# wkentaro/morefusion

Measured on AMD Instinct MI355X. Metric: objects/sec (32^3 voxelize+3D-CNN+ICC refine), higher is better.
Workload: dtype f32; 1 GPU; 1 scene(s) x 8 objects per GPU: singleview_3d Model.predict (ResNet18+PSPNet, 32^3 voxelize, occupancy 3D-CNN, heads; B=8) -> ICC joint refine 100 iters (BASELINE configs[1]+configs[2]); random weights, ICC starts from synthetic perturbed-GT poses; ICC(k) on a second HIP stream, event-ordered after network(k), beside network(k+1); objects_per_gpu=8, icc_iters=100, parallelism=scene-sharded x1, pose all_gather, stream_priority=none, backbone_memory_format=contiguous

## Files before the change

### include/mfhip.h

```cpp
#ifndef MFHIP_H_
#define MFHIP_H_

#include <stdint.h>

#ifdef __cplusplus
extern "C" {
#endif

typedef void *mfStream_t;

int mf_version(void);
const char *mf_last_error_string(void);

int mf_average_voxelization_3d_fwd(const float *values, const float *points,
                                   const int32_t *batch_indices, int64_t n, int C,
                                   int B, int X, int Y, int Z, float ox, float oy,
                                   float oz, float pitch, float *matrix,
                                   int32_t *counts, int32_t *head, int32_t *link,
                                   int32_t *nan_flag, mfStream_t stream);
int mf_average_voxelization_3d_bwd(const float *gmatrix, const float *points,
                                   const int32_t *batch_indices,
                                   const int32_t *counts, int64_t n, int C, int B,
                                   int X, int Y, int Z, float ox, float oy, float oz,
                                   float pitch, float *gvalues, mfStream_t stream);
// ... 217 lines not shown
int64_t mf_sparse_conv3_bf16_workspace_bytes(int64_t n_points, int32_t B, int32_t D);
int mf_sparse_conv3_bf16_tables(void *ws, int64_t n_points, int32_t B, int32_t D, int64_t *out7);
int mf_sparse_conv3_bf16_index(const float *points, const int32_t *batch_indices, int64_t n, int32_t B, int32_t D,
                               void *ws, mfStream_t stream);
int mf_sparse_conv3_bf16_pack(const float *W, int32_t Cout, int32_t Cs, int32_t w_cin, int32_t c_off, void *Wp, void *Wq,
                              mfStream_t stream);
int mf_sparse_conv3_bf16_unpack_dw(const float *dWp, int32_t Cout, int32_t Cs, int32_t w_cin, int32_t c_off, float *dW,
                                   mfStream_t stream);
int mf_sparse_conv3_bf16_reduce(const void *C, const float *dense, const float *bias, void *ws, int64_t n_points,
                                int32_t B, int32_t D, int32_t Cout, int32_t relu, void *out, mfStream_t stream);
int mf_sparse_conv3_bf16_gather_dy(const void *dz, void *ws, int64_t n_points, int32_t B, int32_t D, int32_t Cout,
                                   void *dYg, mfStream_t stream);
int mf_linear_bf16_tiles(const void *A, int32_t lda, const void *W, int64_t w_group_stride, int32_t ldw,
                         const int32_t *tile_group, void *out, int32_t ldo, int32_t M, int32_t N, int32_t K,
                         int32_t out_f32, mfStream_t stream);
int mf_linear_wgrad_bf16_ranges(const void *dY, int32_t ldy, const void *A, int32_t lda, float *dW,
                                int64_t w_group_stride, int32_t ldc, const int32_t *m_range, int32_t groups, int32_t N,
                                int32_t K, mfStream_t stream);
int mf_conv3d_k4s2_bf16_pack_cols(const float *W, int32_t Cout, int32_t Cin, int32_t w_cin, int32_t c_off, void *W2,
                                  mfStream_t stream);
int mf_conv3d_k4s2_bf16_col2im(const void *T, int32_t B, int32_t D, int32_t Cin, void *dx, mfStream_t stream);
int mf_average_voxelization_rows_bf16_fwd(const void *values, int64_t ldv, const float *points,
                                          const int32_t *batch_indices, int64_t n, int32_t C, int32_t B, int32_t D,
                                          const int32_t *counts, const int32_t *head, const int32_t *link,
                                          const int32_t *rowmap, void *A, int64_t lda, mfStream_t stream);
int mf_average_voxelization_rows_bf16_bwd(const void *dA, int64_t lda, const float *points,
                                          const int32_t *batch_indices, const int32_t *counts, const int32_t *rowmap,
                                          int64_t n, int32_t C, int32_t B, int32_t D, void *gvalues, int64_t ldg,
                                          mfStream_t stream);

int mf_average_voxelization_cl_bf16_fwd(const void *values, int64_t ldv, const float *points,
                                        const int32_t *batch_indices, int64_t n, int32_t C, int32_t B, int32_t D,
                                        void *x, int64_t ldx, int32_t *counts, int32_t *head, int32_t *link,
                                        mfStream_t stream);
int mf_average_voxelization_cl_bf16_bwd(const void *gx, int64_t ldx, const float *points, const int32_t *batch_indices,
                                        const int32_t *counts, int64_t n, int32_t C, int32_t B, int32_t D,
                                        void *gvalues, int64_t ldg, mfStream_t stream);
int mf_interpolate_voxel_grid_cl_bf16_fwd(const void *vox, const float *points, const int32_t *batch_indices,
                                          int64_t n, int B, int C, int X, int Y, int Z, void *out, int64_t ldo,
                                          mfStream_t stream);
int mf_interpolate_voxel_grid_cl_bf16_bwd(const void *gout, int64_t ldg, const float *points,
                                          const int32_t *batch_indices, const int32_t *batch_start, int64_t n, int B,
                                          int C, int X, int Y, int Z, void *gvox, int32_t out_bf16, mfStream_t stream);

int mf_upsample_bilinear_cl_fwd(const void *x, void *y, int32_t B, int32_t H, int32_t W, int32_t Ho, int32_t Wo,
                                int32_t C, int32_t bf16, mfStream_t stream);
int mf_upsample_bilinear_cl_split_fwd(const float *x, void *y, int32_t B, int32_t H, int32_t W, int32_t Ho, int32_t Wo,
                                      int32_t C, int32_t ldy, int32_t los, mfStream_t stream);
int mf_split_bf16(const float *x, int64_t sb, int64_t sc, int64_t sh, int64_t sw, int32_t B, int32_t C, int32_t H,
                  int32_t W, void *y, int32_t ldy, int32_t los, mfStream_t stream);
int mf_upsample2x_tapsum_fwd(const float *z, const float *bias, const float *slope, int32_t act, float *y32,
                             int32_t ld32, void *ys, int32_t lds, int32_t los, int32_t B, int32_t H, int32_t W, int32_t C,
                             mfStream_t stream);
int mf_upsample_bilinear_cl_bwd(const void *gy, void *gx, int32_t B, int32_t H, int32_t W, int32_t Ho, int32_t Wo,
                                int32_t C, int32_t bf16, mfStream_t stream);
int mf_upsample_bilinear_cf_fwd(const void *x, void *y, int64_t BC, int32_t H, int32_t W, int32_t Ho, int32_t Wo,
                                int32_t bf16, mfStream_t stream);
int mf_upsample_bilinear_cf_bwd(const void *gy, void *gx, int64_t BC, int32_t H, int32_t W, int32_t Ho, int32_t Wo,
                                int32_t bf16, mfStream_t stream);
int mf_prelu_fwd(const void *x, const float *slope, void *y, int64_t n, int32_t bf16, mfStream_t stream);
int mf_rgb_normalize(const void *rgb, int32_t u8, const float *mean3, const float *std3, float *out, int64_t npix,
                     mfStream_t stream);
int mf_bn_act_fwd(const void *x, const void *identity, const float *mean, const float *var, const float *weight,
                  const float *bias, float eps, void *y, int64_t n, int32_t C, int64_t HW, int32_t channels_last,
                  int32_t relu, int32_t bf16, mfStream_t stream);
int mf_backbone2d_last_path(void);
int64_t mf_prelu_bwd_workspace_floats(int64_t n);
int mf_prelu_bwd(const void *x, const void *dy, const float *slope, void *dx, float *dslope, float *ws, int64_t n,
                 int32_t bf16, mfStream_t stream);

int mf_gemm_bf16_last_tile(void);

int mf_gemm_bf16_nt_plan(int32_t mode, int64_t M, int32_t N, int32_t K, int32_t groups, int32_t table,
                         int64_t dgrad_rows, int32_t may_split, int32_t have_ws, int32_t *tile, int32_t *S);
int mf_gemm_bf16_tn_plan(int32_t Ni, int32_t Nj, int32_t ldc, int64_t rows, int32_t groups, int32_t ranges,
                         int32_t conv, int32_t split, int32_t *form, int32_t *default_split, int32_t *finish);

int mf_psp_tail_rows_bf16_fwd(const void *u2, const int64_t *pix, int32_t B, int32_t P, int32_t H, int32_t W, void *rows,
                              mfStream_t stream);
int mf_psp_tail_rows_bf16_bwd(const void *grows, const int64_t *pix, int32_t B, int32_t P, int32_t H, int32_t W,
                              float *acc, void *gu2, mfStream_t stream);

int mf_confidence_loss_fwd(const float *add, const float *conf, int32_t B, int32_t P, float lambda, float *loss,
                           int32_t *cnt, mfStream_t stream);
int mf_confidence_loss_bwd(const float *add, const float *conf, const int32_t *cnt, const float *gloss, int32_t B,
                           int32_t P, float lambda, float *dadd, float *dconf, mfStream_t stream);

int mf_pose_epilogue_train_fwd(const float *orot, const float *otrn, const float *ocnf, const int64_t *class_id,
                               const float *pts, const float *origin, const float *pitch, int32_t B, int32_t P,
                               int32_t n_fg, float *rot, float *trans, float *conf, mfStream_t stream);
int mf_pose_epilogue_train_bwd(const float *orot, const float *ocnf, const int64_t *class_id, const float *pitch,
                               const float *grot, const float *gtrans, const float *gconf, int32_t B, int32_t P,
                               int32_t n_fg, float *drot, float *dtrn, float *dcnf, mfStream_t stream);
int mf_transformation_matrix_fwd(const float *q, const float *t, int64_t n, float *T, mfStream_t stream);
int mf_transformation_matrix_bwd(const float *q, const float *gT, int64_t n, float *gq, float *gt, mfStream_t stream);
int mf_point_prep(const float *points_cam, const float *values, const float *origin, const float *pitch,
                  int32_t B, int32_t P, int32_t Cv, float center, float *pts, float *tc4, float *x_rows,
                  int32_t *batch_indices, mfStream_t stream);
int mf_pose_epilogue(const float *heads_out, int64_t ldo, int32_t np4, const int64_t *class_id,
                     const float *pts, const float *origin, const float *pitch, int32_t B, int32_t P, int32_t n_fg,
                     float *rot, float *trans, float *conf, mfStream_t stream);

#define MF_PCDNET_WS_BUFFERS 12
#define MF_PCDNET_MAX_FG 256
int32_t mf_pcdnet_workspace_offsets(int32_t B, int32_t P, int32_t n_fg, int64_t *offsets);
int64_t mf_pcdnet_workspace_bytes(int32_t B, int32_t P, int32_t n_fg);
// ... 214 lines not shown
```

### morefusion_amd/_lib.py

```python
import ctypes
import os

import torch

_HERE = os.path.dirname(os.path.abspath(__file__))
SO_PATH = os.path.join(_HERE, os.path.basename(os.environ.get("MF_LIBMFHIP", "libmfhip.so")))
_lib = None

_p = ctypes.c_void_p
_i = ctypes.c_int32
_i64 = ctypes.c_int64
_f = ctypes.c_float
_d = ctypes.c_double


class IccBatch(ctypes.Structure):

    _fields_ = [
        ("pts4", _p), ("obj_off", _p), ("scene_off", _p), ("obj_scene", _p),
        ("pitch", _p), ("origin", _p), ("grid_target", _p), ("grid_ne", _p),
        ("n_objects", _i), ("n_scenes", _i), ("n_points", _i), ("dim", _i), ("max_scene_objects", _i),
        ("voxel_threshold", _f), ("sdf_offset", _f), ("grid_ne_binary", _i), ("flags", _i),
    ]

# ... 78 lines not shown
    "mf_linear_bf16": ([_p, _i64, _i, _p, _i64, _i, _p, _i64, _p, _i64] + [_i] * 8 + [_p], _i),
    "mf_linear_wgrad_bf16": ([_p, _i64, _i, _p, _i64, _i, _p, _i64, _i, _p] + [_i] * 5 + [_p], _i),
    "mf_conv3d_k4s2_pack_bf16": ([_p] + [_i] * 4 + [_p, _p, _p], _i),
    "mf_conv3d_k4s2_bf16_fwd": ([_p, _p, _p, _p] + [_i] * 6 + [_p], _i),
    "mf_conv3d_k4s2_bf16_dgrad": ([_p, _p, _p] + [_i] * 6 + [_p], _i),
    "mf_conv3d_k4s2_bf16_wgrad_workspace_bytes": ([_i] * 3, _i64),
    "mf_conv3d_k4s2_bf16_wgrad_default_split": ([_i] * 4, _i),
    "mf_conv3d_k4s2_bf16_wgrad": ([_p, _p, _p, _p] + [_i] * 7 + [_p], _i),
    "mf_conv3d_bf16_pack": ([_p] + [_i] * 5 + [_p, _p, _p, _p], _i),
    "mf_conv3d_bf16_fwd": ([_p, _p, _p, _p] + [_i] * 11 + [_p], _i),
    "mf_conv3d_bf16_fwd_workspace_bytes": ([_i] * 8, _i64),
    "mf_conv3d_bf16_fwd_ws": ([_p, _p, _p, _p, _p, _i64] + [_i] * 11 + [_p], _i),
    "mf_conv2d_split_pack": ([_p] + [_i] * 3 + [_p, _p], _i),
    "mf_conv2d_split_workspace_bytes": ([_i] * 8, _i64),
    "mf_conv2d_split_fwd": ([_p, _p, _p, _p, _i, _p, _i, _p, _i, _p, _i, _i, _p, _i64] + [_i] * 8 + [_p], _i),
    "mf_conv3d_k4s2_split_pack": ([_p] + [_i] * 4 + [_p, _p], _i),
    "mf_conv3d_k4s2_split_workspace_bytes": ([_i] * 4, _i64),
    "mf_conv3d_k4s2_split_fwd": ([_p, _p, _p, _i, _p, _i, _p, _i, _i, _p, _i64] + [_i] * 4 + [_p], _i),
    "mf_linear_split_pack": ([_p, _i64] + [_i] * 6 + [_p, _p], _i),
    "mf_linear_split_workspace_bytes": ([_i64, _i, _i], _i64),
    "mf_linear_split_fwd": ([_p, _i, _p, _p, _i, _p, _i, _p, _i, _i, _p, _i64] + [_i] * 3 + [_p], _i),
    "mf_sparse_conv3d_k4s2_points_cl_split_fwd": ([_p, _i64, _p, _p, _i64, _f, _f, _f, _f, _p, _p, _p, _p, _p, _p] + [_i] * 6 + [_p], _i),
    "mf_interpolate_voxel_grid_cl_split_fwd": ([_p, _p, _p, _i64, _i, _i, _i, _i, _i, _p, _i64, _i64, _p], _i),
    "mf_conv3d_k3_narrow_bf16_pack_elems": ([_i], _i64),
    "mf_conv3d_k3_narrow_bf16_pack": ([_p] + [_i] * 5 + [_p, _p], _i),
    "mf_conv3d_k3_narrow_bf16": ([_p, _p, _p, _p] + [_i] * 6 + [_p], _i),
    "mf_conv3d_bf16_wgrad_workspace_bytes": ([_i] * 4, _i64),
    "mf_wgrad_split": ([_i64, _i64, _i64], _i),
    "mf_linear_wgrad_bf16_default_split": ([_i64, _i, _i, _i], _i),
    "mf_conv3d_bf16_wgrad_default_split": ([_i] * 5, _i),
    "mf_conv3d_bf16_wgrad": ([_p, _p, _p, _p] + [_i] * 11 + [_p], _i),
    "mf_sparse_conv3_bf16_max_rows": ([_i64], _i64),
    "mf_sparse_conv3_bf16_workspace_bytes": ([_i64, _i, _i], _i64),
    "mf_sparse_conv3_bf16_tables": ([_p, _i64, _i, _i, _p], _i),
    "mf_sparse_conv3_bf16_index": ([_p, _p, _i64, _i, _i, _p, _p], _i),
    "mf_sparse_conv3_bf16_pack": ([_p, _i, _i, _i, _i, _p, _p, _p], _i),
    "mf_sparse_conv3_bf16_unpack_dw": ([_p, _i, _i, _i, _i, _p, _p], _i),
    "mf_sparse_conv3_bf16_reduce": ([_p, _p, _p, _p, _i64, _i, _i, _i, _i, _p, _p], _i),
    "mf_sparse_conv3_bf16_gather_dy": ([_p, _p, _i64, _i, _i, _i, _p, _p], _i),
    "mf_linear_bf16_tiles": ([_p, _i, _p, _i64, _i, _p, _p, _i, _i, _i, _i, _i, _p], _i),
    "mf_linear_wgrad_bf16_ranges": ([_p, _i, _p, _i, _p, _i64, _i, _p, _i, _i, _i, _p], _i),
    "mf_conv3d_k4s2_bf16_pack_cols": ([_p, _i, _i, _i, _i, _p, _p], _i),
    "mf_conv3d_k4s2_bf16_col2im": ([_p, _i, _i, _i, _p, _p], _i),
    "mf_average_voxelization_rows_bf16_fwd": ([_p, _i64, _p, _p, _i64, _i, _i, _i, _p, _p, _p, _p, _p, _i64, _p], _i),
    "mf_average_voxelization_rows_bf16_bwd": ([_p, _i64, _p, _p, _p, _p, _i64, _i, _i, _i, _p, _i64, _p], _i),
    "mf_average_voxelization_cl_bf16_fwd": ([_p, _i64, _p, _p, _i64, _i, _i, _i, _p, _i64, _p, _p, _p, _p], _i),
    "mf_average_voxelization_cl_bf16_bwd": ([_p, _i64, _p, _p, _p, _i64, _i, _i, _i, _p, _i64, _p], _i),
    "mf_interpolate_voxel_grid_cl_bf16_fwd": ([_p, _p, _p, _i64, _i, _i, _i, _i, _i, _p, _i64, _p], _i),
    "mf_interpolate_voxel_grid_cl_bf16_bwd": ([_p, _i64, _p, _p, _p, _i64, _i, _i, _i, _i, _i, _p, _i, _p], _i),
    "mf_upsample_bilinear_cl_fwd": ([_p, _p] + [_i] * 7 + [_p], _i),
    "mf_upsample_bilinear_cl_split_fwd": ([_p, _p] + [_i] * 8 + [_p], _i),
    "mf_upsample2x_tapsum_fwd": ([_p, _p, _p, _i, _p, _i, _p] + [_i] * 6 + [_p], _i),
    "mf_split_bf16": ([_p, _i64, _i64, _i64, _i64] + [_i] * 4 + [_p, _i, _i, _p], _i),
    "mf_upsample_bilinear_cl_bwd": ([_p, _p] + [_i] * 7 + [_p], _i),
    "mf_upsample_bilinear_cf_fwd": ([_p, _p, _i64] + [_i] * 5 + [_p], _i),
    "mf_upsample_bilinear_cf_bwd": ([_p, _p, _i64] + [_i] * 5 + [_p], _i),
    "mf_prelu_fwd": ([_p, _p, _p, _i64, _i, _p], _i),
    "mf_rgb_normalize": ([_p, _i, _p, _p, _p, _i64, _p], _i),
    "mf_bn_act_fwd": ([_p, _p, _p, _p, _p, _p, _f, _p, _i64, _i, _i64, _i, _i, _i, _p], _i),
    "mf_backbone2d_last_path": ([], _i),
    "mf_prelu_bwd_workspace_floats": ([_i64], _i64),
    "mf_prelu_bwd": ([_p, _p, _p, _p, _p, _p, _i64, _i, _p], _i),
    "mf_gemm_bf16_last_tile": ([], _i),
    "mf_gemm_bf16_nt_plan": ([_i, _i64, _i, _i, _i, _i, _i64, _i, _i, _p, _p], _i),
    "mf_gemm_bf16_tn_plan": ([_i, _i, _i, _i64, _i, _i, _i, _i, _p, _p, _p], _i),
    "mf_psp_tail_rows_bf16_fwd": ([_p, _p, _i, _i, _i, _i, _p, _p], _i),
    "mf_psp_tail_rows_bf16_bwd": ([_p, _p, _i, _i, _i, _i, _p, _p, _p], _i),
    "mf_confidence_loss_fwd": ([_p, _p, _i, _i, _f, _p, _p, _p], _i),
    "mf_confidence_loss_bwd": ([_p, _p, _p, _p, _i, _i, _f, _p, _p, _p], _i),
    "mf_pose_epilogue_train_fwd": ([_p, _p, _p, _p, _p, _p, _p, _i, _i, _i, _p, _p, _p, _p], _i),
    "mf_pose_epilogue_train_bwd": ([_p, _p, _p, _p, _p, _p, _p, _i, _i, _i, _p, _p, _p, _p], _i),
    "mf_transformation_matrix_fwd": ([_p, _p, _i64, _p, _p], _i),
    "mf_transformation_matrix_bwd": ([_p, _p, _i64, _p, _p, _p], _i),
    "mf_point_prep": ([_p, _p, _p, _p, _i, _i, _i, _f, _p, _p, _p, _p, _p], _i),
    "mf_pose_epilogue": ([_p, _i64, _i, _p, _p, _p, _p, _i, _i, _i, _p, _p, _p, _p], _i),
    "mf_psp_tail_fwd": ([_p, _i64, _i64, _i64, _i64, _p, _p, _p, _p, _p, _p] + [_i] * 4 + [_p, _p], _i),
    "mf_valid_pixel_order": ([_p, _i, _i, _p, _p, _p], _i),
    "mf_instance_stats": ([_p, _p, _i, _i, _p, _i, _p, _p], _i),
    "mf_instance_crops": ([_p, _p, _p, _i, _i, _d, _d, _d, _d, _p, _p, _i, _i, _i, _p, _p, _p, _p], _i),
    "mf_occmap_regrid": ([ctypes.POINTER(OccTree), ctypes.POINTER(OccTree), _p], _i),
    "mf_occmap_bounds": ([_p, _p, _i64, _p, _i, _p, _i, _p, _p], _i),
    "mf_occmap_raycast": ([_p, _p, _i64, _p, _i, _p, _f, _f, _f, _p, _p], _i),
    "mf_occmap_count_hits": ([_p, _i64, _p, _i, _p, _p], _i),
    "mf_occmap_apply": ([_p, _i, _i64, _i, _p], _i),
    "mf_occmap_extract": ([_p, _i, _p, _p, _p] + [_i] * 4 + [_p] * 6, _i),
    "mf_occtrack_workspace_bytes": ([_i] * 3, _i64),
    "mf_occtrack_stats_elems": ([_i, _i], _i64),
    "mf_occtrack_transform": ([_p, _p, _i64, _p, _p], _i),
    "mf_occtrack_render": ([_p, _p, _p, _f, _f, _f, _p, _p, _i, _i, _i, _p, _p, _p, _p], _i),
    "mf_occtrack_overlap": ([_p, _p, _i, _i, _p, _i, _p, _i, _p, _p], _i),
    "mf_occtrack_assign": ([_p, _p] + [_i] * 7 + [_d, _d] + [_p] * 5, _i),
    "mf_occtrack_relabel": ([_p, _p, _i, _i, _p, _i, _p, _i] + [_p] * 5, _i),
    "mf_occtrack_clean": ([_p] + [_i] * 4 + [_p, _p, _p], _i),
    "mf_occtrack_merge": ([_p, _p, _i, _i, _p, _i, _p, _p, _p], _i),
    "mf_icpreg_workspace_bytes": ([_i64, _i64, _i64], _i64),
    "mf_icpreg_bounds": ([_p, _p, _i, _d, _p, _p, _p], _i),
    "mf_icpreg_prepare": ([_p, _p, _i, _d, _p, _p, _p, _i64, _p, _p, _i64, _d, _i64] + [_p] * 7, _i),
    "mf_icpreg_run": ([ctypes.POINTER(IcpRegBatch), _p], _i),
    "mf_meshsdf_workspace_bytes": ([_i64], _i64),
    "mf_meshsdf_prepare": ([ctypes.POINTER(MeshSdfBatch), _i64, _p], _i),
    "mf_meshsdf_query": ([ctypes.POINTER(MeshSdfBatch), _p], _i),
    "mf_render_workspace_bytes": ([_i64] * 4, _i64),
    "mf_render_setup": ([_p, _i64, _p], _i),
    "mf_render_raster": ([_p, _i64, _p], _i),
    "mf_render_resolve": ([_p, _i64, _p], _i),
    "mf_full_grids": ([_p] * 5 + [_i, _i64, _i, _p, _p, _p], _i),
# ... 89 lines not shown
```

### morefusion_amd/csrc/backbone2d.hip

```cpp
#include "mf_common.h"

namespace {

__device__ __forceinline__ float up_scale(int in, int out) { return out > 1 ? (float)(in - 1) / (float)(out - 1) : 0.0f; }

struct UpSrc { int y0, x0, yp, xp; float h0, h1, w0, w1; };
__device__ __forceinline__ UpSrc up_src(int oy, int ox, int H, int W, int Ho, int Wo) {
  UpSrc s;
  const float sy = up_scale(H, Ho) * (float)oy, sx = up_scale(W, Wo) * (float)ox;
  s.y0 = (int)sy; s.x0 = (int)sx;
  s.yp = s.y0 < H - 1 ? 1 : 0; s.xp = s.x0 < W - 1 ? 1 : 0;
  s.h1 = sy - (float)s.y0; s.h0 = 1.0f - s.h1; s.w1 = sx - (float)s.x0; s.w0 = 1.0f - s.w1;
  return s;
}

template <bool BF16>
__device__ __forceinline__ void load8(const void *p, int64_t idx, float v[8]) {
  if (BF16) {
    const uint4 w = *reinterpret_cast<const uint4 *>(reinterpret_cast<const uint16_t *>(p) + idx);
    const uint32_t d[4] = {w.x, w.y, w.z, w.w};
#pragma unroll
    for (int i = 0; i < 4; ++i) { v[2 * i] = mf::bf16_lo(d[i]); v[2 * i + 1] = mf::bf16_hi(d[i]); }
  } else {
    const float4 a = *reinterpret_cast<const float4 *>(reinterpret_cast<const float *>(p) + idx);
// ... 85 lines not shown
  if (i >= (int64_t)B * Ho * Wo * C8) return;
  const int c8 = (int)(i % C8);
  const int64_t pix = i / C8;
  const int ox = (int)(pix % Wo), oy = (int)((pix / Wo) % Ho), b = (int)(pix / ((int64_t)Wo * Ho));
  const int C = 8 * C8;
  const int64_t ldz = 9 * (int64_t)C;
  const float *zb = z + (int64_t)b * H * W * ldz + 8 * c8;
  float acc[8] = {0.0f, 0.0f, 0.0f, 0.0f, 0.0f, 0.0f, 0.0f, 0.0f};
#pragma unroll
  for (int ky = 0; ky < 3; ++ky) {
    const int qy = oy + ky - 1;
    if (qy < 0 || qy >= Ho) continue;
#pragma unroll
    for (int kx = 0; kx < 3; ++kx) {
      const int qx = ox + kx - 1;
      if (qx < 0 || qx >= Wo) continue;
      const UpSrc s = up_src(qy, qx, H, W, Ho, Wo);
      const float *p = zb + ((int64_t)s.y0 * W + s.x0) * ldz + (ky * 3 + kx) * C;
      float a00[8], a01[8], a10[8], a11[8];
      load8<false>(p, 0, a00);
      load8<false>(p, s.xp * ldz, a01);
      load8<false>(p, s.yp * W * ldz, a10);
      load8<false>(p, ((int64_t)s.yp * W + s.xp) * ldz, a11);
#pragma unroll
      for (int k = 0; k < 8; ++k)
        acc[k] += s.h0 * (s.w0 * a00[k] + s.w1 * a01[k]) + s.h1 * (s.w0 * a10[k] + s.w1 * a11[k]);
    }
  }
  float bv[8];
  load8<false>(bias, 8 * c8, bv);
  const float sl = act == 2 ? *slope : 0.0f;
#pragma unroll
  for (int k = 0; k < 8; ++k) {
    acc[k] += bv[k];
    if (act) acc[k] = acc[k] > 0.0f ? acc[k] : sl * acc[k];
  }
  if (y32) store8<false>(y32, pix * ld32 + 8 * c8, acc);
  if (ys) store8_split(ys, pix * lds + 8 * c8, los, acc);
}

__global__ __launch_bounds__(256) void k_split_bf16(const float *__restrict__ x, int64_t sb, int64_t sc, int64_t sh,
                                                    int64_t sw, int B, int C8, int H, int W, uint16_t *__restrict__ y,
                                                    int ldy, int los) {
  const int64_t i = (int64_t)blockIdx.x * blockDim.x + threadIdx.x;
  if (i >= (int64_t)B * H * W * C8) return;
  const int c8 = (int)(i % C8);
  const int64_t pix = i / C8;
  const int px = (int)(pix % W), py = (int)((pix / W) % H), b = (int)(pix / ((int64_t)W * H));
  const float *src = x + b * sb + py * sh + px * sw + 8 * c8 * sc;
  float v[8];
#pragma unroll
  for (int k = 0; k < 8; ++k) v[k] = src[k * sc];
  store8_split(y, pix * ldy + 8 * c8, los, v);
}

template <bool BF16>
__global__ __launch_bounds__(256) void k_up_bwd(const void *__restrict__ gy, void *__restrict__ gx, int B, int H, int W,
                                                int Ho, int Wo, int C8) {
  const int64_t i = (int64_t)blockIdx.x * blockDim.x + threadIdx.x;
  const int64_t total = (int64_t)B * H * W * C8;
  if (i >= total) return;
  const int c8 = (int)(i % C8);
  const int64_t pix = i / C8;
  const int ix = (int)(pix % W), iy = (int)((pix / W) % H), b = (int)(pix / ((int64_t)W * H));
  const float ssy = up_scale(H, Ho), ssx = up_scale(W, Wo);
  int oy_lo = 0, oy_hi = Ho - 1, ox_lo = 0, ox_hi = Wo - 1;
  if (ssy > 0.0f) {
    oy_lo = max(0, (int)floorf((float)(iy - 1) / ssy));
    oy_hi = min(Ho - 1, (int)ceilf((float)(iy + 1) / ssy));
  }
  if (ssx > 0.0f) {
    ox_lo = max(0, (int)floorf((float)(ix - 1) / ssx));
    ox_hi = min(Wo - 1, (int)ceilf((float)(ix + 1) / ssx));
  }
  const int C = 8 * C8;
  float acc[8] = {0, 0, 0, 0, 0, 0, 0, 0};
  for (int oy = oy_lo; oy <= oy_hi; ++oy) {
    const float sy = ssy * (float)oy;
    const int y0 = (int)sy;
    const int yp = y0 < H - 1 ? 1 : 0;
    const float h1 = sy - (float)y0, h0 = 1.0f - h1;
    if (!(y0 == iy || y0 + yp == iy)) continue;
    float wy = 0.0f;
    if (y0 == iy) wy += h0;
    if (y0 + yp == iy) wy += h1;
    for (int ox = ox_lo; ox <= ox_hi; ++ox) {
      const float sx = ssx * (float)ox;
      const int x0 = (int)sx;
      const int xp = x0 < W - 1 ? 1 : 0;
      const float w1 = sx - (float)x0, w0 = 1.0f - w1;
      if (!(x0 == ix || x0 + xp == ix)) continue;
      float wx = 0.0f;
      if (x0 == ix) wx += w0;
      if (x0 + xp == ix) wx += w1;
      float g[8];
      load8<BF16>(gy, (((int64_t)b * Ho + oy) * Wo + ox) * C + 8 * c8, g);
      const float w = wy * wx;
#pragma unroll
      for (int k = 0; k < 8; ++k) acc[k] += w * g[k];
    }
  }
  store8<BF16>(gx, pix * C + 8 * c8, acc);
}


constexpr int kUpT = 8;
// ... 293 lines not shown
  hipStream_t stream = (hipStream_t)stream_;
  if ((int64_t)B * Ho * Wo * C == 0) return 0;
  if (C % 8 || H < 1 || W < 1 || (((uintptr_t)x | (uintptr_t)y) & 15)) return bad2d("upsample_bilinear_cl: C % 8 == 0, aligned");
  const int64_t total = (int64_t)B * Ho * Wo * (C / 8);
  const unsigned nb = (unsigned)((total + 255) / 256);
  if (bf16) hipLaunchKernelGGL(k_up_fwd<true>, dim3(nb), dim3(256), 0, stream, x, y, B, H, W, Ho, Wo, C / 8);
  else hipLaunchKernelGGL(k_up_fwd<false>, dim3(nb), dim3(256), 0, stream, x, y, B, H, W, Ho, Wo, C / 8);
  return mf::check_launch("mf_upsample_bilinear_cl_fwd");
}

extern "C" int mf_upsample_bilinear_cl_split_fwd(const float *x, void *y, int32_t B, int32_t H, int32_t W, int32_t Ho,
                                                 int32_t Wo, int32_t C, int32_t ldy, int32_t los, mfStream_t stream_) {
  hipStream_t stream = (hipStream_t)stream_;
  if ((int64_t)B * Ho * Wo * C == 0) return 0;
  if (C % 8 || ldy % 8 || los % 8 || los < C || ldy < los + C || H < 1 || W < 1 ||
      (((uintptr_t)x | (uintptr_t)y) & 15))
    return bad2d("upsample_bilinear_cl_split: C, ldy, los % 8 == 0, los >= C, ldy >= los + C, aligned");
  const int64_t total = (int64_t)B * Ho * Wo * (C / 8);
  hipLaunchKernelGGL(k_up_fwd_split, dim3((unsigned)((total + 255) / 256)), dim3(256), 0, stream, x, (uint16_t *)y, B, H,
                     W, Ho, Wo, C / 8, ldy, los);
  return mf::check_launch("mf_upsample_bilinear_cl_split_fwd");
}

extern "C" int mf_upsample2x_tapsum_fwd(const float *z, const float *bias, const float *slope, int32_t act, float *y32,
                                        int32_t ld32, void *ys, int32_t lds, int32_t los, int32_t B, int32_t H, int32_t W,
                                        int32_t C, mfStream_t stream_) {
  hipStream_t stream = (hipStream_t)stream_;
  if ((int64_t)B * H * W * C == 0) return 0;
  if (C < 8 || C % 8 || H < 1 || W < 1 || B < 0 || !bias || (!y32 && !ys) || act < 0 || act > 2 || (act == 2 && !slope))
    return bad2d("upsample2x_tapsum: C % 8 == 0, a bias, at least one output, act 0 / 1 / 2 (PReLU needs its slope)");
  if ((y32 && (ld32 < C || ld32 % 8)) || (ys && (lds % 8 || los % 8 || los < C || lds < los + C)))
    return bad2d("upsample2x_tapsum: pitches >= C and multiples of 8; lo plane inside the row");
  if (((uintptr_t)z | (uintptr_t)bias | (uintptr_t)y32 | (uintptr_t)ys) & 15 || ((uintptr_t)slope & 3))
    return bad2d("upsample2x_tapsum: 16-byte aligned operands");
  const int64_t total = (int64_t)B * 4 * H * W * (C / 8);
  if ((total + 255) / 256 >= (1ll << 31)) return bad2d("upsample2x_tapsum: too many output elements for one launch");
  hipLaunchKernelGGL(k_up_tapsum, dim3((unsigned)((total + 255) / 256)), dim3(256), 0, stream, z, bias, slope, act, y32,
                     ld32, (uint16_t *)ys, lds, los, B, H, W, C / 8);
  return mf::check_launch("mf_upsample2x_tapsum_fwd");
}

extern "C" int mf_split_bf16(const float *x, int64_t sb, int64_t sc, int64_t sh, int64_t sw, int32_t B, int32_t C,
                             int32_t H, int32_t W, void *y, int32_t ldy, int32_t los, mfStream_t stream_) {
  hipStream_t stream = (hipStream_t)stream_;
  if ((int64_t)B * C * H * W == 0) return 0;
  if (C % 8 || ldy % 8 || los % 8 || los < C || ldy < los + C || ((uintptr_t)y & 15))
    return bad2d("split_bf16: C, ldy, los % 8 == 0, los >= C, ldy >= los + C, aligned output");
  const int64_t total = (int64_t)B * H * W * (C / 8);
  hipLaunchKernelGGL(k_split_bf16, dim3((unsigned)((total + 255) / 256)), dim3(256), 0, stream, x, sb, sc, sh, sw, B,
                     C / 8, H, W, (uint16_t *)y, ldy, los);
  return mf::check_launch("mf_split_bf16");
}

extern "C" int mf_upsample_bilinear_cl_bwd(const void *gy, void *gx, int32_t B, int32_t H, int32_t W, int32_t Ho,
                                           int32_t Wo, int32_t C, int32_t bf16, mfStream_t stream_) {
  hipStream_t stream = (hipStream_t)stream_;
  if ((int64_t)B * H * W * C == 0) return 0;
  if (C % 8 || (((uintptr_t)gx | (uintptr_t)gy) & 15)) return bad2d("upsample_bilinear_cl: C % 8 == 0, aligned");
  const int64_t total = (int64_t)B * H * W * (C / 8);
  const unsigned nb = (unsigned)((total + 255) / 256);
  if (C % 64 == 0 && (int64_t)H * W <= 64 && (int64_t)Ho * Wo >= 16 * (int64_t)H * W) {
    const dim3 grid((unsigned)(H * W), (unsigned)(C / 64), (unsigned)B);
    g_b2d_last_path = kPathUpSmall;
    if (bf16) hipLaunchKernelGGL(k_up_bwd_small<true>, grid, dim3(512), 0, stream, gy, gx, H, W, Ho, Wo, C);
    else hipLaunchKernelGGL(k_up_bwd_small<false>, grid, dim3(512), 0, stream, gy, gx, H, W, Ho, Wo, C);
    return mf::check_launch("mf_upsample_bilinear_cl_bwd");
  }
  if (bf16 && C % 64 == 0 && H >= kUpT && W >= kUpT) {
    const float sy = Ho > 1 ? (float)(H - 1) / (float)(Ho - 1) : 0.0f, sx = Wo > 1 ? (float)(W - 1) / (float)(Wo - 1) : 0.0f;
    const int rows = sy > 0.0f ? (int)ceilf((float)(kUpT + 1) / sy) + 3 : Ho, cols = sx > 0.0f ? (int)ceilf((float)(kUpT + 1) / sx) + 3 : Wo;
    const size_t lds = (size_t)rows * cols * 128;
    if (lds <= 64 * 1024) {
      const int tx = (W + kUpT - 1) / kUpT, ty = (H + kUpT - 1) / kUpT;
      g_b2d_last_path = kPathUpTile;
      hipLaunchKernelGGL(k_up_bwd_tile_bf16, dim3((unsigned)(tx * ty), (unsigned)(C / 64), (unsigned)B), dim3(512), lds, stream,
                         (const uint16_t *)gy, (uint16_t *)gx, H, W, Ho, Wo, C, tx);
      return mf::check_launch("mf_upsample_bilinear_cl_bwd");
    }
  }
  g_b2d_last_path = kPathUpDirect;
  if (bf16) hipLaunchKernelGGL(k_up_bwd<true>, dim3(nb), dim3(256), 0, stream, gy, gx, B, H, W, Ho, Wo, C / 8);
  else hipLaunchKernelGGL(k_up_bwd<false>, dim3(nb), dim3(256), 0, stream, gy, gx, B, H, W, Ho, Wo, C / 8);
  return mf::check_launch("mf_upsample_bilinear_cl_bwd");
}


extern "C" int mf_upsample_bilinear_cf_fwd(const void *x, void *y, int64_t BC, int32_t H, int32_t W, int32_t Ho,
                                           int32_t Wo, int32_t bf16, mfStream_t stream_) {
  hipStream_t stream = (hipStream_t)stream_;
  const int64_t total = BC * Ho * Wo;
  if (total == 0) return 0;
  const unsigned nb = (unsigned)((total + 255) / 256);
  if (bf16) hipLaunchKernelGGL(k_up_fwd_cf<true>, dim3(nb), dim3(256), 0, stream, x, y, BC, H, W, Ho, Wo);
  else hipLaunchKernelGGL(k_up_fwd_cf<false>, dim3(nb), dim3(256), 0, stream, x, y, BC, H, W, Ho, Wo);
  return mf::check_launch("mf_upsample_bilinear_cf_fwd");
}

extern "C" int mf_upsample_bilinear_cf_bwd(const void *gy, void *gx, int64_t BC, int32_t H, int32_t W, int32_t Ho,
                                           int32_t Wo, int32_t bf16, mfStream_t stream_) {
  hipStream_t stream = (hipStream_t)stream_;
  const int64_t total = BC * H * W;
  if (total == 0) return 0;
  const unsigned nb = (unsigned)((total + 255) / 256);
  if (bf16) hipLaunchKernelGGL(k_up_bwd_cf<true>, dim3(nb), dim3(256), 0, stream, gy, gx, BC, H, W, Ho, Wo);
  else hipLaunchKernelGGL(k_up_bwd_cf<false>, dim3(nb), dim3(256), 0, stream, gy, gx, BC, H, W, Ho, Wo);
  return mf::check_launch("mf_upsample_bilinear_cf_bwd");
// ... 73 lines not shown
```

### morefusion_amd/models/backbone2d.py

```python

import os

import torch
import torch.nn as nn
import torch.nn.functional as F

from . import ops2d


class BasicBlock(nn.Module):
    def __init__(self, in_channels, out_channels, stride, dilate, residual_conv=False):
        super().__init__()
        self.conv1 = nn.Conv2d(in_channels, out_channels, 3, stride, padding=dilate,
                               dilation=dilate, bias=False)
        self.conv2 = nn.Conv2d(out_channels, out_channels, 3, 1, padding=dilate,
                               dilation=dilate, bias=False)
        self.residual_conv = (
            nn.Conv2d(in_channels, out_channels, 1, stride, bias=False) if residual_conv else None)

    def forward(self, x):
        h = self.conv2(F.relu(self.conv1(x)))
        residual = x if self.residual_conv is None else self.residual_conv(x)
        return F.relu(h + residual)


class ResBlock(nn.Sequential):
    def __init__(self, n_layer, in_channels, out_channels, stride, dilate, residual_conv=True):
        blocks = [BasicBlock(in_channels, out_channels, stride, 1, residual_conv=residual_conv)]
        for _ in range(n_layer - 1):
            blocks.append(BasicBlock(out_channels, out_channels, 1, dilate))
        super().__init__(*blocks)


SPLIT_MIN_BATCH = {"res4_res5": 4, "psp_up1": 1, "up2": 4}
CONV_BEFORE_RESIZE_MIN_BATCH = {"up1": 4, "up2": 4}


def _split_path(module, x, group):
    D = x.shape[2]
    return (module.split_bf16 and x.is_cuda and x.dtype == torch.float32 and not module.training
            and not torch.is_grad_enabled() and not torch.is_autocast_enabled()
            and x.shape[0] >= SPLIT_MIN_BATCH[group] and x.shape[3] == D and D > 0 and D & (D - 1) == 0)


def _block_split(blk, xs, x32, need32=True, needs=True):
    if blk.residual_conv is not None:
        r, _ = ops2d.conv_split(xs, blk.residual_conv)
    else:
        r = x32
    _, t = ops2d.conv_split(xs, blk.conv1, act=1, out32=False, outs=True)
    y32, ys = ops2d.conv_split(t, blk.conv2, res=r, act=1, out32=need32, outs=needs)
    return ys, y32


class ResNet18(nn.Module):

    split_bf16 = True

    mean_rgb = (0.485, 0.456, 0.406)
    std_rgb = (0.229, 0.224, 0.225)

    def __init__(self):
        super().__init__()
        self.conv1 = nn.Conv2d(3, 64, 7, 2, 3, bias=False)
        self.res2 = ResBlock(2, 64, 64, 1, 1, residual_conv=False)
        self.res3 = ResBlock(2, 64, 128, 2, 1)
        self.res4 = ResBlock(2, 128, 256, 1, 2)
        self.res5 = ResBlock(2, 256, 512, 1, 4)
        self.register_buffer("mean", torch.tensor(self.mean_rgb).view(1, 3, 1, 1))
        self.register_buffer("std", torch.tensor(self.std_rgb).view(1, 3, 1, 1))

    def forward(self, x):
        h = (x / 255.0 - self.mean) / self.std
        h = self.conv1(h)
        h = F.max_pool2d(h, 3, 2, 1)
        h = self.res3(self.res2(h))
        if _split_path(self, h, "res4_res5"):
            blocks = list(self.res4) + list(self.res5)
            xs, x32 = ops2d.to_split(h), None
            for i, blk in enumerate(blocks):
                nxt = blocks[i + 1] if i + 1 < len(blocks) else None
                xs, x32 = _block_split(blk, xs, x32, need32=nxt is None or nxt.residual_conv is None,
                                       needs=nxt is not None)
            return x32.permute(0, 3, 1, 2)
        return self.res5(self.res4(h))


class _ConvBlock(nn.Module):

    def __init__(self, cin, cout, k, stride=1, pad=0, dilate=1, activate=True):
        super().__init__()
        self.conv = nn.Conv2d(cin, cout, k, stride, padding=pad, dilation=dilate, bias=False)
        self.bn = nn.BatchNorm2d(cout, eps=1e-5)
        self.activate = activate

    def forward(self, x):
        h = self.conv(x)
        if ops2d.bn_act_supported(h, self.bn):
            return ops2d.bn_act(h, self.bn, relu=self.activate)
        h = self.bn(h)
        return F.relu(h) if self.activate else h


class _ResBody(nn.Module):
    def __init__(self, cin, cout, stride, dilate):
        super().__init__()
        self.conv1 = _ConvBlock(cin, cout, 3, stride, pad=dilate, dilate=dilate)
        self.conv2 = _ConvBlock(cout, cout, 3, 1, pad=dilate, dilate=dilate, activate=False)

    def forward(self, x):
        return self.conv2(self.conv1(x))


class _ResUnit(nn.Module):

    def __init__(self, cin, cout, stride, dilate, resize):
        super().__init__()
        self.body = _ResBody(cin, cout, stride, dilate)
        self.identity_conv = _ConvBlock(cin, cout, 1, stride, activate=False) if resize else None

    def forward(self, x):
        identity = x if self.identity_conv is None else self.identity_conv(x)
        last = self.body.conv2
        h = last.conv(self.body.conv1(x))
        if ops2d.bn_act_supported(h, last.bn) and identity.shape == h.shape:
            return ops2d.bn_act(h, last.bn, identity=identity, relu=True)
        return F.relu(last.bn(h) + identity)


class _InitBlock(nn.Module):
    def __init__(self):
        super().__init__()
        self.conv = _ConvBlock(3, 64, 7, 2, pad=3)

    def forward(self, x):
        return F.max_pool2d(self.conv(x), 3, 2, 1)
# ... 77 lines not shown
            pooled = torch.matmul(Pm.t(), x.float().permute(0, 2, 3, 1).reshape(B, H * W, C)).to(x.dtype)
        out, o = [], 0
        for size in self.sizes:
            n_y, n_x = (H - H // size) // (H // size) + 1, (W - W // size) // (W // size) + 1
            out.append(pooled[:, o:o + n_y * n_x].transpose(1, 2).reshape(B, C, n_y, n_x)
                       .contiguous(memory_format=torch.channels_last))
            o += n_y * n_x
        return out

    def branches(self, x):
        H, W = x.shape[2:]
        hs = []
        for pooled, conv in zip(self._pooled(x), self.convs):
            h = conv(pooled).contiguous(memory_format=torch.channels_last)
            hs.append(ops2d.upsample_bilinear(h, (H, W)) if ops2d.supported(h) else
                      F.interpolate(h, (H, W), mode="bilinear", align_corners=True))
        return hs

    def forward(self, x):
        return F.relu(self.bottleneck(torch.cat(self.branches(x) + [x], dim=1)))


class PSPUpsample(nn.Module):
    def __init__(self, in_channels, out_channels):
        super().__init__()
        self.conv = nn.Conv2d(in_channels, out_channels, 3, 1, padding=1)
        self.prelu = nn.PReLU()

    def forward(self, x):
        H, W = x.shape[2:]
        if ops2d.supported(x):
            h = ops2d.upsample_bilinear(x, (H * 2, W * 2))
        else:
            h = F.interpolate(x, (H * 2, W * 2), mode="bilinear", align_corners=True)
        h = self.conv(h)
        if ops2d.supported(h, self.prelu.weight.numel()):
            return ops2d.prelu(h, self.prelu.weight)
        return self.prelu(h)


class PSPNetExtractor(nn.Module):

    def __init__(self):
        super().__init__()
        self.psp = PSPModule(512, 1024, [1, 2, 3, 6])
        self.up1 = PSPUpsample(1024, 256)
        self.up2 = PSPUpsample(256, 64)
        self.up3 = PSPUpsample(64, 64)
        self.conv1 = nn.Conv2d(64, 32, 1)

    bf16_tail_kernels = True
    split_bf16 = True
    conv_before_resize = os.environ.get("MF_CONV_BEFORE_RESIZE", "1") != "0"

    def _conv_first(self, x, layer):
        return self.conv_before_resize and x.shape[0] >= CONV_BEFORE_RESIZE_MIN_BATCH[layer]

    def __getstate__(self):
        state = dict(self.__dict__)
        state.pop("_tail_pack", None)
        return state

    def forward(self, x):
        h = F.dropout(self.psp(x), 0.3, self.training)
        h = F.dropout(self.up1(h), 0.15, self.training)
        h = F.dropout(self.up2(h), 0.15, self.training)
        h = self.up3(h)
        return F.log_softmax(self.conv1(h), dim=1)

    def forward_sampled(self, x, pix, plan=None):
        h = F.dropout(self.psp(x), 0.3, self.training)
        h = F.dropout(self.up1(h), 0.15, self.training)
        u2 = F.dropout(self.up2(h), 0.15, self.training)
        if (plan is None and self.bf16_tail_kernels and u2.is_cuda and u2.shape[1] == 64 and self.conv1.out_channels == 32
                and self.up3.prelu.weight.numel() == 1 and torch.is_autocast_enabled()
                and torch.get_autocast_dtype("cuda") == torch.bfloat16 and os.environ.get("MF_TORCH_TAIL") != "1"):
            B, P = pix.shape
            return self._tail_rows_bf16(u2, pix).reshape(B, P, -1).transpose(1, 2)
        taps = plan if plan is not None else self.plan(pix, x.shape[2], x.shape[3])
        return self._tail(u2, taps)

    def _tail_rows_bf16(self, u2, pix):
        from ..contrib.singleview_3d.models import bf16_ops as K
        n = pix.numel()
        rows = ops2d.tail_rows(u2, pix)
        pre = K.Linear.apply(rows, self.up3.conv.weight, self.up3.conv.bias, False)
        h = ops2d._PReLU.apply(pre.view(1, 1, n, 64), self.up3.prelu.weight).view(n, 64)
        z = K.Linear.apply(h, self.conv1.weight, self.conv1.bias, False)
        return F.log_softmax(z.float(), dim=1)

    def forward_sampled_rows(self, x, pix):
        from .. import _lib
        if _split_path(self, x, "psp_up1") and self.up1.prelu.weight.numel() == 1:
            slope2 = self.up2.prelu.weight.detach()
            if slope2.numel() == 1 and self._conv_first(x, "up2"):
                _, hs = self._psp_up1_split(x, need32=False, needs=True)
                z = ops2d.conv_taps_split(hs, self.up2.conv)
                u2, _ = ops2d.upsample_tapsum(z, self.up2.conv.bias.detach(), act=2, slope=slope2)
                u2 = u2.permute(0, 3, 1, 2)
            elif slope2.numel() == 1 and _split_path(self, x, "up2"):
                h, _ = self._psp_up1_split(x)
                us = ops2d.upsample_split(h, 2 * h.shape[1], 2 * h.shape[2])
                u2, _ = ops2d.conv_split(us, self.up2.conv, act=2, slope=slope2)
                u2 = u2.permute(0, 3, 1, 2)
            else:
                h, _ = self._psp_up1_split(x)
                u2 = self.up2(h.permute(0, 3, 1, 2))
# ... 103 lines not shown
```

### morefusion_amd/models/ops2d.py

```python
import os

import torch

from .. import _lib


def _dense(x):
    if x.is_contiguous(memory_format=torch.channels_last) and x.shape[1] % 8 == 0 and x.shape[1] > 1:
        return x, torch.channels_last
    if x.is_contiguous():
        return x, torch.contiguous_format
    if x.stride(1) == 1 and x.shape[1] % 8 == 0:
        return x.contiguous(memory_format=torch.channels_last), torch.channels_last
    return x.contiguous(), torch.contiguous_format


def supported(x, n_slope=1):
    if not (x.is_cuda and x.dim() == 4 and x.dtype in (torch.float32, torch.bfloat16) and n_slope == 1):
        return False
    if x.numel() % 8:
        return False
    dense = x.is_contiguous() or x.is_contiguous(memory_format=torch.channels_last)
    return not dense or x.data_ptr() % 16 == 0

# ... 110 lines not shown
            raise ValueError("tail_rows: the map must have 64 channels")
        u = u2.detach().to(torch.bfloat16).contiguous(memory_format=torch.channels_last)
        pixc = pix.reshape(-1).to(torch.int64).contiguous()
        P = pix.shape[1]
        rows = torch.empty((B * P, 576), dtype=torch.bfloat16, device=u.device)
        _lib.check(_lib.lib().mf_psp_tail_rows_bf16_fwd(u.data_ptr(), pixc.data_ptr(), B, P, H, W, rows.data_ptr(),
                                                        _lib.stream_ptr()), "mf_psp_tail_rows_bf16_fwd")
        ctx.save_for_backward(pixc)
        ctx.geom = (B, P, H, W, u2.dtype)
        return rows

    @staticmethod
    def backward(ctx, grows):
        (pixc,) = ctx.saved_tensors
        B, P, H, W, dtype = ctx.geom
        g = grows.to(torch.bfloat16).contiguous()
        acc = torch.empty((B, H, W, 64), dtype=torch.float32, device=g.device)
        gu = torch.empty((B, 64, H, W), dtype=torch.bfloat16, device=g.device, memory_format=torch.channels_last)
        _lib.check(_lib.lib().mf_psp_tail_rows_bf16_bwd(g.data_ptr(), pixc.data_ptr(), B, P, H, W, acc.data_ptr(),
                                                        gu.data_ptr(), _lib.stream_ptr()), "mf_psp_tail_rows_bf16_bwd")
        return gu.to(dtype), None


def tail_rows(u2, pix):
    return _TailRows.apply(u2, pix)


def _autocast_dtype(x):
    if x.is_cuda and torch.is_autocast_enabled() and torch.get_autocast_dtype("cuda") == torch.bfloat16:
        return x.to(torch.bfloat16)
    return x


def upsample_bilinear(x, size):
    return _Upsample.apply(_autocast_dtype(x), int(size[0]), int(size[1]))


def prelu(x, slope):
    return _PReLU.apply(_autocast_dtype(x), slope)



def split_pack(conv):
    w = conv.weight
    key = (w.data_ptr(), w._version)
    hit = conv.__dict__.get("_split_pack")
    if hit is not None and hit[0] == key:
        return hit[1]
    Cout, Cin, k, _ = w.shape
    wp = torch.empty((Cout, k * k, 3 * Cin), dtype=torch.bfloat16, device=w.device)
    wf = w.detach().float().contiguous()
    _lib.check(_lib.lib().mf_conv2d_split_pack(wf.data_ptr(), Cout, Cin, k, wp.data_ptr(), _lib.stream_ptr()),
               "mf_conv2d_split_pack")
    if not torch.cuda.is_current_stream_capturing():
        conv.__dict__["_split_pack"] = (key, wp)
    return wp


def to_split(x, out=None, c_off=0, los=None):
    B, C, H, W = x.shape
    if out is None:
        out, los = torch.empty((B, H, W, 2 * C), dtype=torch.bfloat16, device=x.device), C
    _lib.check(_lib.lib().mf_split_bf16(x.data_ptr(), *x.stride(), B, C, H, W, out[..., c_off:].data_ptr(),
                                        out.shape[3], los, _lib.stream_ptr()), "mf_split_bf16")
    return out


def upsample_split(x_cl, Ho, Wo, out=None, c_off=0, los=None):
    B, H, W, C = x_cl.shape
    if out is None:
        out, los = torch.empty((B, Ho, Wo, 2 * C), dtype=torch.bfloat16, device=x_cl.device), C
    _lib.check(_lib.lib().mf_upsample_bilinear_cl_split_fwd(x_cl.data_ptr(), out[..., c_off:].data_ptr(), B, H, W, Ho, Wo,
                                                            C, out.shape[3], los, _lib.stream_ptr()),
               "mf_upsample_bilinear_cl_split_fwd")
    return out


def conv_split(xs, conv, res=None, act=0, slope=None, out32=True, outs=False):
    B, D, D2, C2 = xs.shape
    Cout, Cin, k, _ = conv.weight.shape
    if D2 != D or C2 != 2 * Cin or not xs.is_contiguous():
        raise ValueError(f"conv_split: a contiguous square split map [B, D, D, {2 * Cin}] is required, got {tuple(xs.shape)}")
    stride, pad, dil = conv.stride[0], conv.padding[0], conv.dilation[0]
    Do = (D + 2 * pad - dil * (k - 1) - 1) // stride + 1
    L = _lib.lib()
    wp = split_pack(conv)
    y32 = torch.empty((B, Do, Do, Cout), dtype=torch.float32, device=xs.device) if out32 else None
    ys = torch.empty((B, Do, Do, 2 * Cout), dtype=torch.bfloat16, device=xs.device) if outs else None
    nws = L.mf_conv2d_split_workspace_bytes(B, Cin, Cout, D, k, stride, pad, dil)
    ws = torch.empty((nws,), dtype=torch.uint8, device=xs.device) if nws > 0 else None
    bias = conv.bias.detach() if conv.bias is not None else None
    _lib.check(L.mf_conv2d_split_fwd(xs.data_ptr(), wp.data_ptr(), _lib.ptr(bias), _lib.ptr(res),
                                     res.stride(2) if res is not None else 0, _lib.ptr(slope), act, _lib.ptr(y32), Cout,
                                     _lib.ptr(ys), 2 * Cout, Cout, _lib.ptr(ws), nws, B, Cin, Cout, D, k, stride, pad, dil,
                                     _lib.stream_ptr()), "mf_conv2d_split_fwd")
    return y32, ys



def tap_pack(conv):
    w = conv.weight
    key = (w.data_ptr(), w._version)
    hit = conv.__dict__.get("_tap_pack")
    if hit is not None and hit[0] == key:
        return hit[1]
    Cout, Cin, k, k2 = w.shape
    if k != 3 or k2 != 3:
        raise ValueError("tap_pack: a 3 x 3 convolution is required")
    wf = w.detach().float().permute(2, 3, 0, 1).reshape(9 * Cout, Cin).contiguous()
    wp = torch.empty((9 * Cout, 1, 3 * Cin), dtype=torch.bfloat16, device=w.device)
    _lib.check(_lib.lib().mf_conv2d_split_pack(wf.data_ptr(), 9 * Cout, Cin, 1, wp.data_ptr(), _lib.stream_ptr()),
               "mf_conv2d_split_pack")
    if not (w.is_cuda and torch.cuda.is_current_stream_capturing()):
        conv.__dict__["_tap_pack"] = (key, wp)
    return wp


def conv_taps_split(xs, conv):
    B, D, D2, C2 = xs.shape
    Cout, Cin = conv.weight.shape[:2]
    if D2 != D or C2 != 2 * Cin or not xs.is_contiguous():
        raise ValueError(f"conv_taps_split: a contiguous square split map [B, D, D, {2 * Cin}] is required, got {tuple(xs.shape)}")
    if conv.stride[0] != 1 or conv.padding[0] != 1 or conv.dilation[0] != 1:
        raise ValueError("conv_taps_split: stride 1, padding 1, dilation 1")
    L = _lib.lib()
    wp = tap_pack(conv)
    N = 9 * Cout
    z = torch.empty((B, D, D, N), dtype=torch.float32, device=xs.device)
    nws = L.mf_conv2d_split_workspace_bytes(B, Cin, N, D, 1, 1, 0, 1)
    ws = torch.empty((nws,), dtype=torch.uint8, device=xs.device) if nws > 0 else None
    _lib.check(L.mf_conv2d_split_fwd(xs.data_ptr(), wp.data_ptr(), None, None, 0, None, 0, z.data_ptr(), N, None, 0, 0,
                                     _lib.ptr(ws), nws, B, Cin, N, D, 1, 1, 0, 1, _lib.stream_ptr()),
               "mf_conv2d_split_fwd")
    return z


def upsample_tapsum(z, bias, act=0, slope=None, out32=True, outs=False):
    B, H, W, N = z.shape
    if N % 72 or z.dtype != torch.float32 or not z.is_contiguous():
        raise ValueError(f"upsample_tapsum: contiguous fp32 [B, H, W, 9 C] with C % 8 == 0 is required, got {tuple(z.shape)}")
    C = N // 9
    _lib.require_gpu(z, bias)
    y32 = torch.empty((B, 2 * H, 2 * W, C), dtype=torch.float32, device=z.device) if out32 else None
    ys = torch.empty((B, 2 * H, 2 * W, 2 * C), dtype=torch.bfloat16, device=z.device) if outs else None
    _lib.check(_lib.lib().mf_upsample2x_tapsum_fwd(z.data_ptr(), bias.data_ptr(), _lib.ptr(slope), act, _lib.ptr(y32), C,
                                                   _lib.ptr(ys), 2 * C, C, B, H, W, C, _lib.stream_ptr()),
               "mf_upsample2x_tapsum_fwd")
    return y32, ys
```

Measured before the change: 1928 objects/sec.

## Fuse stem maxpool with bf16 split packing and run res2/res3 on split path

```diff
diff --git a/include/mfhip.h b/include/mfhip.h
--- a/include/mfhip.h
+++ b/include/mfhip.h
@@ -293,6 +293,8 @@
 int mf_upsample2x_tapsum_fwd(const float *z, const float *bias, const float *slope, int32_t act, float *y32,
                              int32_t ld32, void *ys, int32_t lds, int32_t los, int32_t B, int32_t H, int32_t W, int32_t C,
                              mfStream_t stream);
+int mf_maxpool3s2_split_fwd(const float *x, int64_t sb, int64_t sc, int64_t sh, int64_t sw, int32_t B, int32_t C,
+                            int32_t H, int32_t W, float *y32, void *ys, mfStream_t stream);
 int mf_upsample_bilinear_cl_bwd(const void *gy, void *gx, int32_t B, int32_t H, int32_t W, int32_t Ho, int32_t Wo,
                                 int32_t C, int32_t bf16, mfStream_t stream);
 int mf_upsample_bilinear_cf_fwd(const void *x, void *y, int64_t BC, int32_t H, int32_t W, int32_t Ho, int32_t Wo,
diff --git a/morefusion_amd/_lib.py b/morefusion_amd/_lib.py
--- a/morefusion_amd/_lib.py
+++ b/morefusion_amd/_lib.py
@@ -154,6 +154,7 @@
     "mf_upsample_bilinear_cl_split_fwd": ([_p, _p] + [_i] * 8 + [_p], _i),
     "mf_upsample2x_tapsum_fwd": ([_p, _p, _p, _i, _p, _i, _p] + [_i] * 6 + [_p], _i),
     "mf_split_bf16": ([_p, _i64, _i64, _i64, _i64] + [_i] * 4 + [_p, _i, _i, _p], _i),
+    "mf_maxpool3s2_split_fwd": ([_p, _i64, _i64, _i64, _i64] + [_i] * 4 + [_p, _p, _p], _i),
     "mf_upsample_bilinear_cl_bwd": ([_p, _p] + [_i] * 7 + [_p], _i),
     "mf_upsample_bilinear_cf_fwd": ([_p, _p, _i64] + [_i] * 5 + [_p], _i),
     "mf_upsample_bilinear_cf_bwd": ([_p, _p, _i64] + [_i] * 5 + [_p], _i),
diff --git a/morefusion_amd/csrc/backbone2d.hip b/morefusion_amd/csrc/backbone2d.hip
--- a/morefusion_amd/csrc/backbone2d.hip
+++ b/morefusion_amd/csrc/backbone2d.hip
@@ -161,6 +161,53 @@
 #pragma unroll
   for (int k = 0; k < 8; ++k) v[k] = src[k * sc];
   store8_split(y, pix * ldy + 8 * c8, los, v);
+}
+
+constexpr int kMpPix = 16, kMpCh = 64, kMpPitch = kMpCh + 1;
+
+__global__ __launch_bounds__(256) void k_maxpool3s2_split(const float *__restrict__ x, int64_t sb, int64_t sc, int64_t sh,
+                                                          int64_t sw, int C, int H, int W, int Ho, int Wo, int strips,
+                                                          float *__restrict__ y32, uint16_t *__restrict__ ys) {
+  __shared__ float s_t[kMpPix * kMpPitch];
+  const int strip = blockIdx.x % strips, oy = blockIdx.x / strips;
+  const int c0 = blockIdx.y * kMpCh, b = blockIdx.z;
+  const float *xb = x + b * sb;
+  for (int i = threadIdx.x; i < kMpPix * kMpCh; i += 256) {
+    int p, c;
+    if (sc == 1) { c = i % kMpCh; p = i / kMpCh; }
+    else { p = i % kMpPix; c = i / kMpPix; }
+    const int ox = strip * kMpPix + p;
+    float m = -INFINITY;
+    if (ox < Wo && c0 + c < C) {
+      const float *xc = xb + (c0 + c) * sc;
+#pragma unroll
+      for (int ky = 0; ky < 3; ++ky) {
+        const int iy = 2 * oy + ky - 1;
+        if (iy < 0 || iy >= H) continue;
+#pragma unroll
+        for (int kx = 0; kx < 3; ++kx) {
+          const int ix = 2 * ox + kx - 1;
+          if (ix < 0 || ix >= W) continue;
+          const float v = xc[iy * sh + ix * sw];
+          if (v > m || v != v) m = v;
+        }
+      }
+    }
+    s_t[p * kMpPitch + c] = m;
+  }
+  __syncthreads();
+  if (threadIdx.x < kMpPix * (kMpCh / 8)) {
+    const int c8 = threadIdx.x % (kMpCh / 8), p = threadIdx.x / (kMpCh / 8);
+    const int ox = strip * kMpPix + p, ch = c0 + 8 * c8;
+    if (ox < Wo && ch < C) {
+      float v[8];
+#pragma unroll
+      for (int k = 0; k < 8; ++k) v[k] = s_t[p * kMpPitch + 8 * c8 + k];
+      const int64_t pix = ((int64_t)b * Ho + oy) * Wo + ox;
+      if (y32) store8<false>(y32, pix * C + ch, v);
+      if (ys) store8_split(ys, pix * 2 * C + ch, C, v);
+    }
+  }
 }
 
 template <bool BF16>
@@ -560,6 +607,19 @@
   return mf::check_launch("mf_split_bf16");
 }
 
+extern "C" int mf_maxpool3s2_split_fwd(const float *x, int64_t sb, int64_t sc, int64_t sh, int64_t sw, int32_t B,
+                                       int32_t C, int32_t H, int32_t W, float *y32, void *ys, mfStream_t stream_) {
+  hipStream_t stream = (hipStream_t)stream_;
+  if ((int64_t)B * C * H * W == 0) return 0;
+  if (B < 0 || B > 65535 || C < 8 || C % 8 || H < 1 || W < 1 || !x || (!y32 && !ys) ||
+      (((uintptr_t)y32 | (uintptr_t)ys) & 15))
+    return bad2d("maxpool3s2_split: C % 8 == 0, B <= 65535, at least one output, aligned outputs");
+  const int Ho = (H - 1) / 2 + 1, Wo = (W - 1) / 2 + 1, strips = (Wo + kMpPix - 1) / kMpPix;
+  hipLaunchKernelGGL(k_maxpool3s2_split, dim3((unsigned)(strips * Ho), (unsigned)((C + kMpCh - 1) / kMpCh), (unsigned)B),
+                     dim3(256), 0, stream, x, sb, sc, sh, sw, C, H, W, Ho, Wo, strips, y32, (uint16_t *)ys);
+  return mf::check_launch("mf_maxpool3s2_split_fwd");
+}
+
 extern "C" int mf_upsample_bilinear_cl_bwd(const void *gy, void *gx, int32_t B, int32_t H, int32_t W, int32_t Ho,
                                            int32_t Wo, int32_t C, int32_t bf16, mfStream_t stream_) {
   hipStream_t stream = (hipStream_t)stream_;
diff --git a/morefusion_amd/models/backbone2d.py b/morefusion_amd/models/backbone2d.py
--- a/morefusion_amd/models/backbone2d.py
+++ b/morefusion_amd/models/backbone2d.py
@@ -32,7 +32,7 @@
         super().__init__(*blocks)
 
 
-SPLIT_MIN_BATCH = {"res4_res5": 4, "psp_up1": 1, "up2": 4}
+SPLIT_MIN_BATCH = {"res4_res5": 4, "psp_up1": 1, "up2": 4, "res2_res3": 4}
 CONV_BEFORE_RESIZE_MIN_BATCH = {"up1": 4, "up2": 4}
 
 
@@ -56,6 +56,7 @@
 class ResNet18(nn.Module):
 
     split_bf16 = True
+    front_split = os.environ.get("MF_FRONT_SPLIT", "1") != "0"
 
     mean_rgb = (0.485, 0.456, 0.406)
     std_rgb = (0.229, 0.224, 0.225)
@@ -70,18 +71,27 @@
         self.register_buffer("mean", torch.tensor(self.mean_rgb).view(1, 3, 1, 1))
         self.register_buffer("std", torch.tensor(self.std_rgb).view(1, 3, 1, 1))
 
+    @staticmethod
+    def _blocks_split(blocks, xs, x32):
+        for i, blk in enumerate(blocks):
+            nxt = blocks[i + 1] if i + 1 < len(blocks) else None
+            xs, x32 = _block_split(blk, xs, x32, need32=nxt is None or nxt.residual_conv is None,
+                                   needs=nxt is not None)
+        return x32
+
     def forward(self, x):
         h = (x / 255.0 - self.mean) / self.std
         h = self.conv1(h)
+        if self.front_split and _split_path(self, h, "res2_res3"):
+            x32, xs = ops2d.maxpool_split(h)
+            back = h.shape[0] >= SPLIT_MIN_BATCH["res4_res5"]
+            blocks = list(self.res2) + list(self.res3) + (list(self.res4) + list(self.res5) if back else [])
+            h = self._blocks_split(blocks, xs, x32).permute(0, 3, 1, 2)
+            return h if back else self.res5(self.res4(h))
         h = F.max_pool2d(h, 3, 2, 1)
         h = self.res3(self.res2(h))
         if _split_path(self, h, "res4_res5"):
-            blocks = list(self.res4) + list(self.res5)
-            xs, x32 = ops2d.to_split(h), None
-            for i, blk in enumerate(blocks):
-                nxt = blocks[i + 1] if i + 1 < len(blocks) else None
-                xs, x32 = _block_split(blk, xs, x32, need32=nxt is None or nxt.residual_conv is None,
-                                       needs=nxt is not None)
+            x32 = self._blocks_split(list(self.res4) + list(self.res5), ops2d.to_split(h), None)
             return x32.permute(0, 3, 1, 2)
         return self.res5(self.res4(h))
 
@@ -265,7 +275,6 @@
     bf16_tail_kernels = True
     split_bf16 = True
     conv_before_resize = os.environ.get("MF_CONV_BEFORE_RESIZE", "1") != "0"
-
     def _conv_first(self, x, layer):
         return self.conv_before_resize and x.shape[0] >= CONV_BEFORE_RESIZE_MIN_BATCH[layer]
 
diff --git a/morefusion_amd/models/ops2d.py b/morefusion_amd/models/ops2d.py
--- a/morefusion_amd/models/ops2d.py
+++ b/morefusion_amd/models/ops2d.py
@@ -186,7 +186,7 @@
     wf = w.detach().float().contiguous()
     _lib.check(_lib.lib().mf_conv2d_split_pack(wf.data_ptr(), Cout, Cin, k, wp.data_ptr(), _lib.stream_ptr()),
                "mf_conv2d_split_pack")
-    if not torch.cuda.is_current_stream_capturing():
+    if not (w.is_cuda and torch.cuda.is_current_stream_capturing()):
         conv.__dict__["_split_pack"] = (key, wp)
     return wp
 
@@ -281,3 +281,15 @@
                                                    _lib.ptr(ys), 2 * C, C, B, H, W, C, _lib.stream_ptr()),
                "mf_upsample2x_tapsum_fwd")
     return y32, ys
+
+
+
+def maxpool_split(x, out32=True, outs=True):
+    _lib.require_gpu(x)
+    B, C, H, W = x.shape
+    Ho, Wo = (H - 1) // 2 + 1, (W - 1) // 2 + 1
+    y32 = torch.empty((B, Ho, Wo, C), dtype=torch.float32, device=x.device) if out32 else None
+    ys = torch.empty((B, Ho, Wo, 2 * C), dtype=torch.bfloat16, device=x.device) if outs else None
+    _lib.check(_lib.lib().mf_maxpool3s2_split_fwd(x.data_ptr(), *x.stride(), B, C, H, W, _lib.ptr(y32), _lib.ptr(ys),
+                                                  _lib.stream_ptr()), "mf_maxpool3s2_split_fwd")
+    return y32, ys
```

New measurement: 1985 objects/sec (median of 6 runs). +3.0%, better.
